# kyle-he/gym-comm

Measured on AMD Instinct MI355X. Metric: env-steps/sec (whole node), higher is better.
Workload: dtype int32

## Files before the change

gym-comm_amd/csrc/oc_step_device.h:

```cpp
#pragma once
#include <hip/hip_runtime.h>

#include <type_traits>

#include "../../include/oc_hip.h"
#include "oc_level_host.h"
#include "oc_policy_device.h"

namespace {

#ifdef OC_STAMPS
#define OC_STAMP(k)                                                                  \
  do {                                                                               \
    unsigned long long t_;                                                           \
    __builtin_amdgcn_sched_barrier(0);                                               \
    asm volatile("s_memtime %0\n\ts_waitcnt lgkmcnt(0)" : "=s"(t_)::"memory");     \
    __builtin_amdgcn_sched_barrier(0);                                               \
    oc_tt[(k)] = t_;                                                                 \
  } while (0)
#define OC_STAMP_PARAM , unsigned long long (&oc_tt)[16]
#define OC_STAMP_PASS , oc_tt
#else
#define OC_STAMP(k) do { } while (0)
#define OC_STAMP_PARAM
// ... 63 lines not shown
#define OC_HDR_LOAD(args) const HdrK L {(args).L}
#endif
#undef OC_KF
#undef OC_KA

constexpr int IW_POS = 0x000000FF, IW_CHOP = 0x00000100, IW_GRP = 0x00000E00, IW_HOLD = 0x00007000,
              IW_SEQ = 0x00FF0000, IW_TSET = 0x0F000000;
template <bool DUP>
constexpr int TS = DUP ? 0x7F000000 : IW_TSET;
template <bool DUP>
constexpr int OBJ = IW_GRP | IW_SEQ | TS<DUP>;
template <bool DUP>
__host__ __device__ constexpr int sig_of_type(int t) { return DUP ? (1 << (24 + 2 * t)) : (1 << (24 + t)); }

template <int A, int M, bool DUP>
struct Env {
  int ap[A], ahp[A];
  int iw[M];
  int t, completed, goalcnt, mctr, err;
  int kn[2];
};
template <int A, int M, bool DUP>
constexpr int state_words() { return A + M + 2 + (DUP ? 2 : 0); }

__device__ __forceinline__ int ipos(int w) { return w & IW_POS; }
__device__ __forceinline__ int ichop(int w) { return (w >> 8) & 1; }
__device__ __forceinline__ int igrp(int w) { return (w >> 9) & 7; }
__device__ __forceinline__ int iseq(int w) { return (w >> 16) & 255; }
__device__ __forceinline__ int itset(int w) { return (w >> 24) & 15; }
__device__ __forceinline__ int bfi(int mask, int a, int b) { return (a & mask) | (b & ~mask); }

template <int A, int M, bool DUP>
__device__ __forceinline__ void unpack(Env<A, M, DUP> &e, const int32_t *w) {
#pragma unroll
  for (int a = 0; a < A; a++) {
    e.ap[a] = w[a] & 255;
    e.ahp[a] = (w[a] >> 8) & 15;
  }
#pragma unroll
  for (int i = 0; i < M; i++) e.iw[i] = w[A + i];
  e.t = (w[0] >> 16) & 0xFFFF;
  e.mctr = (w[1] >> 16) & 255;
  e.err = (w[1] >> 24) & 255;
  e.completed = w[A + M];
  e.goalcnt = w[A + M + 1];
  if constexpr (DUP) e.kn[0] = w[A + M + 2], e.kn[1] = w[A + M + 3];
}

template <int A, int M, bool DUP>
__device__ __forceinline__ void pack(const Env<A, M, DUP> &e, int32_t *w) {
#pragma unroll
  for (int a = 0; a < A; a++) w[a] = e.ap[a] | (e.ahp[a] << 8);
  w[0] |= e.t << 16;
  w[1] |= (e.mctr << 16) | (e.err << 24);
#pragma unroll
  for (int i = 0; i < M; i++) w[A + i] = e.iw[i];
  w[A + M] = e.completed;
  w[A + M + 1] = e.goalcnt;
  if constexpr (DUP) w[A + M + 2] = e.kn[0], w[A + M + 3] = e.kn[1];
}

typedef int P;
constexpr int WAIT_VMCNT0 = 0x0F70;
__device__ __forceinline__ int hide(int v) {
  asm("" : "+v"(v));
  return v;
}
__device__ __forceinline__ P sign_of(int d) { return hide(hide(d) >> 31); }
__device__ __forceinline__ P p_z(int a) { return sign_of((int)((unsigned)a - 1u)); }
__device__ __forceinline__ P p_nz(int a) { return sign_of((int)(0u - (unsigned)a)); }
__device__ __forceinline__ P p_eq(int a, int b) { return sign_of((int)((unsigned)(a ^ b) - 1u)); }
__device__ __forceinline__ P p_ne(int a, int b) { return ~p_eq(a, b); }
__device__ __forceinline__ P p_lt(int a, int b) { return sign_of(a - b); }
__device__ __forceinline__ P p_gt(int a, int b) { return p_lt(b, a); }
__device__ __forceinline__ P p_ge(int a, int b) { return ~p_lt(a, b); }
__device__ __forceinline__ P p_le(int a, int b) { return ~p_lt(b, a); }
__device__ __forceinline__ P p_eq_any(int a, int b) { return hide(a == b ? -1 : 0); }
__device__ __forceinline__ P p_gtu_any(unsigned a, unsigned b) { return hide(a > b ? -1 : 0); }
__device__ __forceinline__ P p_geu_any(unsigned a, unsigned b) { return hide(a >= b ? -1 : 0); }
__device__ __forceinline__ P p_ltu_any(unsigned a, unsigned b) { return hide(a < b ? -1 : 0); }
__device__ __forceinline__ P p_bit(int w, unsigned k) { return hide(__builtin_amdgcn_sbfe(w, k, 1u)); }
__device__ __forceinline__ P p_of(bool uniform) { return uniform ? -1 : 0; }
__device__ __forceinline__ int sel(P m, int a, int b) { return (a & m) | (b & ~m); }

__device__ __forceinline__ int iabs(int v) { return v < 0 ? -v : v; }
__device__ __forceinline__ unsigned sad_u32(unsigned a, unsigned b, unsigned c) {
  unsigned r;
  asm("v_sad_u32 %0, %1, %2, %3" : "=v"(r) : "v"(a), "v"(b), "v"(c));
  return r;
}
__device__ __forceinline__ int manhattan(int p, int q) {
  return (int)sad_u32((unsigned)(p & 15), (unsigned)(q & 15), sad_u32((unsigned)(p >> 4), (unsigned)(q >> 4), 0u));
}
__device__ __forceinline__ int px(int p) { return p & 15; }
__device__ __forceinline__ int py(int p) { return p >> 4; }
__device__ __forceinline__ int dense(const Hdr &L, int p) {
  return __mul24(py(p), L.W() - 16) + p;
}
__device__ __forceinline__ int bit128(uint64_t w0, uint64_t w1, int c) {
  const uint64_t v = (c & 64) ? w1 : w0;
  return (int)((v >> (c & 63)) & 1);
}
__device__ __forceinline__ int item_type(const Hdr &L, int i) { return (L.item_types() >> (4 * i)) & 15; }
__device__ __forceinline__ int cell_type(const Hdr &L, int c) {
  if (!L.planes128())
    return (int)((L.cell_lo(0) >> c) & 1) | ((int)((L.cell_hi(0) >> c) & 1) << 1);
  return bit128(L.cell_lo(0), L.cell_lo(1), c) | (bit128(L.cell_hi(0), L.cell_hi(1), c) << 1);
}

#ifdef OC_SPECIALIZED
constexpr bool OC_BORDER_CLOSED = OC_SPEC_HDR.closed_border != 0;
#else
constexpr bool OC_BORDER_CLOSED = false;
#endif

__device__ __forceinline__ double timestep_of(int t, const RunCfg &R) {
  typedef int v2i __attribute__((ext_vector_type(2)));
  const double dt = (double)t;
  const double q0 = dt * R.inv_T;
  const double r = __builtin_fma(-(double)R.T, q0, dt);
  const v2i q = __builtin_bit_cast(v2i, __builtin_fma(r, R.inv_T, q0));
  const P unlimited = p_of(R.T == 0);
  const int hi0 = 0x7FF00000 | (p_z(t) & 0x00080000);
  v2i out;
  out.x = q.x & ~unlimited;
  out.y = sel(unlimited, hi0, q.y);
  return __builtin_bit_cast(double, out);
}


template <int AUX>
struct RowsT {
  __amdgpu_buffer_rsrc_t rsrc;
  int voff;
  int rowbytes;
  __device__ __forceinline__ RowsT(const void *base, int64_t n, int rows, int64_t i, int elem = 4) {
    rsrc = __builtin_amdgcn_make_buffer_rsrc(const_cast<void *>(base), 0, (int)(n * rows * elem), 0x00020000);
    voff = (int)i * elem;
    rowbytes = (int)n * elem;
  }
  __device__ __forceinline__ int ld(int row) const {
    return __builtin_amdgcn_raw_buffer_load_b32(rsrc, voff, row * rowbytes, 0);
  }
  __device__ __forceinline__ void st(int row, int v) const {
    __builtin_amdgcn_raw_buffer_store_b32(v, rsrc, voff, row * rowbytes, AUX);
  }
  __device__ __forceinline__ void st8(int row, int v) const {
    __builtin_amdgcn_raw_buffer_store_b8((char)v, rsrc, voff, row * rowbytes, AUX);
  }
  __device__ __forceinline__ void st_f64(int row, double v) const {
    typedef int v2i __attribute__((ext_vector_type(2)));
    __builtin_amdgcn_raw_buffer_store_b64(__builtin_bit_cast(v2i, v), rsrc, voff, row * rowbytes, AUX);
  }
  __device__ __forceinline__ int soff(int row) const { return row * rowbytes; }
  __device__ __forceinline__ void st_at(int so, int, int v) const {
    __builtin_amdgcn_raw_buffer_store_b32(v, rsrc, voff, so, AUX);
  }
  __device__ __forceinline__ void st8_at(int so, int, int v) const {
    __builtin_amdgcn_raw_buffer_store_b8((char)v, rsrc, voff, so, AUX);
  }
};
template <int AUX, int N>
struct RowsPreT : RowsT<AUX> {
  int so[N > 0 ? N : 1];
  int row0;
  __device__ __forceinline__ RowsPreT(const RowsT<AUX> &rows, int row0_) : RowsT<AUX>(rows), row0(row0_) {
// ... 215 lines not shown
        d_tile[b] = min(d_tile[b], ld.d_tile[k][b] + manhattan(in.ap[b], (int)L.deliv_pos(k)));
    }
  int nchop = 0;
  int mind[B];
#pragma unroll
  for (int b = 0; b < B; b++) mind[b] = 1 << 20;
#pragma unroll
  for (int f = 0; f < 3; f++)
    if (L.chop_mask(f) != 0) {
      const int open = __popc((int)L.chop_mask(f) & ~completed);
      nchop += open;
#pragma unroll
      for (int b = 0; b < B; b++) mind[b] = open ? min(mind[b], ld.d_chop[f][b]) : mind[b];
    }
  int npairs = (int)L.pair_static_max();
  int minpair = npairs ? MAXP : (1 << 20);
  {
    int cur = MAXP;
#pragma unroll
    for (int k = 0; k < MAX_PAIRLK; k++)
      if (k < (int)L.npairlk()) {
        cur = min(cur, ld.d_pair[k]);
        if ((L.pairlk(k) >> 8) & 1) {
          const bool keep = cur != 0;
          npairs += keep ? 1 : 0;
          minpair = keep ? min(minpair, cur) : minpair;
          cur = MAXP;
        }
      }
  }
  int kq_chop[B], kq_pair;
#pragma unroll
  for (int b = 0; b < B; b++) kq_chop[b] = nchop ? (mind[b] + MAXP) + (nchop - 1) * 2 * MAXP : 0;
  kq_pair = nchop ? npairs * MAXP : (npairs ? minpair + (npairs - 1) * MAXP : 0);
  int kq_del[MAX_DELS][B];
#pragma unroll
  for (int k = 0; k < MAX_DELS; k++)
#pragma unroll
    for (int b = 0; b < B; b++) {
      kq_del[k][b] = 0;
      q.del_direct[k][b] = false;
      if (k < (int)L.ndel()) {
        const int d = ld.d_del[k][b] + manhattan(in.ap[b], in.del_p[k]);
        q.del_direct[k][b] = d == 0;
        kq_del[k][b] = d == 0 ? d_tile[b] : d;
      }
    }
#pragma unroll
  for (int b = 0; b < B; b++) q.q_chop[b] = quotient(kq_chop[b], L, inv_max_path);
  q.q_pair = quotient(kq_pair, L, inv_max_path);
#pragma unroll
  for (int k = 0; k < MAX_DELS; k++)
#pragma unroll
    for (int b = 0; b < B; b++) q.q_del[k][b] = (k < (int)L.ndel()) ? quotient(kq_del[k][b], L, inv_max_path) : 0.0;
  q.nchop = nchop;
  q.npairs = npairs;
  OC_STAMP(4);
}

template <int B>
__device__ __forceinline__ void shaping_sum(const Hdr &L, const ShapeIn<B> &in, const ShapeQ<B> &q,
                                            double &s0, double &s1 OC_STAMP_PARAM) {
  double tot[B];
#pragma unroll
  for (int b = 0; b < B; b++) {
    tot[b] = q.nchop ? q.q_chop[b] : 0.0;
    tot[b] = q.npairs ? tot[b] + q.q_pair : tot[b];
  }
#pragma unroll
  for (int k = 0; k < MAX_DELS; k++)
    if (k < (int)L.ndel()) {
      const bool open = !((in.completed >> L.del_bit(k)) & 1);
#pragma unroll
      for (int b = 0; b < B; b++) {
        const double add = !in.del_has[k] ? 2.0 : (q.del_direct[k][b] ? q.q_del[k][b] : q.q_del[k][b] + 1.0);
        tot[b] = open ? tot[b] + add : tot[b];
      }
    }
  s0 = tot[0];
  s1 = B > 1 ? tot[1] : 0.0;
  OC_STAMP(6);
}

template <int A, int M, bool DUP, int PM, bool FLAT>
__device__ __forceinline__ void env_step(const Hdr &L, const RunCfg &R, const uint8_t *__restrict__ dist,
                                         const uint32_t *__restrict__ probe,
                                         Env<A, M, DUP> &e, const int (&act_in)[A], int &reward, int &done, P &done_p,
                                         int &success, ShapeIn<(A < 2 ? A : 2)> &sin,
                                         ShapeLoads<(A < 2 ? A : 2)> &sld OC_STAMP_PARAM) {
  const int W = L.W(), H = L.H();
  const auto pb = [](int w, unsigned k) -> P {
    if constexpr (PM == 2 && FLAT) return __builtin_amdgcn_sbfe(w, k, 1u);
    return p_bit(w, k);
  };
  e.t = min(e.t + 1, 0xFFFF);
  static_assert(OC_ACT_NOOP == 4 && OC_FLOOR == 0 && OC_COUNTER == 1 && OC_CUTBOARD == 2 && OC_DELIVERY == 3, "codes");

  int act[A], np[A], tgt_p[A];
  P moving[A], t_nonfloor[A], t_deliv[A], t_cutb[A];
#pragma unroll
  for (int a = 0; a < A; a++) {
    int c = act_in[a];
    e.err |= p_gtu_any((unsigned)c, 4u) & OC_ERR_ACTION;
    c = (int)min((unsigned)c, 4u);
    act[a] = c;
    moving[a] = p_ne(c, OC_ACT_NOOP);
    int cell;
    P oob = 0;
    if constexpr (OC_BORDER_CLOSED) {
      constexpr uint64_t STEP = 0x0001FFF010ull;
      const int q = e.ap[a] + (int)(int8_t)(STEP >> (8 * c));
      tgt_p[a] = q;
      cell = dense(L, q);
    } else {
      const int dx = (c == OC_ACT_RIGHT) - (c == OC_ACT_LEFT);
      const int dy = (c == OC_ACT_DOWN) - (c == OC_ACT_UP);
      const int qx = px(e.ap[a]) + dx, qy = py(e.ap[a]) + dy;
      oob = ~(p_ltu_any((unsigned)qx, (unsigned)W) & p_ltu_any((unsigned)qy, (unsigned)H));
      e.err |= oob & OC_ERR_OOB;
      const int tx = min(max(qx, 0), W - 1), ty = min(max(qy, 0), H - 1);
      tgt_p[a] = tx | (ty << 4);
      cell = ty * W + tx;
    }
    P lo, hi;
    if (!L.planes128()) {
      lo = pb((int)(L.cell_lo(0) >> cell), 0);
      hi = pb((int)(L.cell_hi(0) >> cell), 0);
    } else {
      lo = -bit128(L.cell_lo(0), L.cell_lo(1), cell);
      hi = -bit128(L.cell_hi(0), L.cell_hi(1), cell);
    }
    t_nonfloor[a] = lo | hi;
    t_deliv[a] = lo & hi;
    t_cutb[a] = hi & ~lo;
    np[a] = sel(t_nonfloor[a] | oob, e.ap[a], tgt_p[a]);
  }
  P ex[A];
#pragma unroll
  for (int a = 0; a < A; a++) ex[a] = -1;
#pragma unroll
  for (int i = 0; i < A; i++)
#pragma unroll
    for (int j = i + 1; j < A; j++) {
      const P same = p_eq(np[i], np[j]);
      const P i_stays = p_eq(np[i], e.ap[i]) & moving[i];
      const P j_stays = p_eq(np[j], e.ap[j]) & moving[j];
      const P swap = p_eq(e.ap[i], np[j]) & p_eq(e.ap[j], np[i]);
      const P block_i = sel(same, ~i_stays, swap);
      const P block_j = sel(same, i_stays | ~j_stays, swap);
      ex[i] &= ~block_i;
      ex[j] &= ~block_j;
    }

  const P play = p_of(PM == 2 ? R.play != 0 : PM == 1);
#pragma unroll
  for (int a = 0; a < A; a++) {
    const P acting = ex[a] & moving[a];
    const int pa = e.ap[a];
    const int tp = tgt_p[a];
    const int held_g = A == 2 ? hide(e.ahp[a] - 1) : e.ahp[a] - 1;
    const P holding = A == 2 ? ~hide(held_g >> 31) : p_nz(e.ahp[a]);
    const int hold_code = (a + 1) << 12;
    int held_or = 0, tgt_or = 0;
    P mine[M], tgt[M];
#pragma unroll
    for (int i = 0; i < M; i++) {
      const int w = e.iw[i];
      const int u = item_type(L, i) != OC_PLATE ? (w ^ IW_CHOP) : w;
      mine[i] = A == 2 ? pb(w, 12 + a) : p_eq(w & IW_HOLD, hold_code);
      tgt[i] = p_eq(w & (IW_HOLD | IW_POS), tp);
      held_or |= mine[i] & u;
      tgt_or |= tgt[i] & u;
    }
    const P tgt_any = p_nz(tgt_or);
    P held_multi;
    if constexpr (DUP) {
      int nm = 0;
#pragma unroll
      for (int i = 0; i < M; i++) nm -= mine[i];
      held_multi = p_gt(nm, 1);
    } else {
      held_multi = p_nz(held_or & IW_TSET & ((held_or & IW_TSET) - (1 << 24)));
    }
    const P held_fresh = pb(held_or, 8);
    const P any_fresh = pb(held_or | tgt_or, 8);
    const P two_plates = p_nz((held_or & tgt_or) & sig_of_type<DUP>(OC_PLATE));
    const P at_deliv = t_deliv[a];
    const P nf = acting & t_nonfloor[a];
    const P do_move = acting & ~t_nonfloor[a];
    const P nfh = nf & holding & ~at_deliv, nfe = nf & ~holding & ~at_deliv;
    const P do_deliver = nf & holding & at_deliv & held_multi & ~held_fresh;
    const P mergeable = ~(two_plates | any_fresh);
    const P do_merge = nfh & tgt_any & mergeable;
    const P chop_here = t_cutb[a] & ~held_multi & held_fresh & ~play;
    const P do_chop = nfh & ~tgt_any & chop_here;
    const P do_drop = nfh & ~tgt_any & ~chop_here;
    const P chop_there = nfe & tgt_any & play & t_cutb[a] & pb(tgt_or, 8);
    const P do_pick = nfe & tgt_any & ~chop_there & p_of(!((R.allergic >> a) & 1));
    const P put = do_deliver | do_drop | (do_merge & play);
    const P take = (do_merge & ~play) | do_pick;
    const int newg = (int)min((unsigned)held_g, (unsigned)igrp(tgt_or));
    int objf;
    if constexpr (DUP) {
      const int newsig = (held_or & TS<true>) + (tgt_or & TS<true>);
      const int seq4 = M + e.mctr;
      int kf = 0;
#pragma unroll
      for (int j = 0; j < MAX_NAMES; j++)
        if (j < (int)L.nnames()) {
          const P hit = p_eq(newsig >> 24, (int)L.name_sig(j));
          const int sh = 4 * (j & 7);
          const int cur = (e.kn[j >> 3] >> sh) & 15;
          kf = sel(hit, cur, kf);
          const P enter = hit & p_z(cur);
          e.kn[j >> 3] |= enter & do_merge & ((seq4 + 1) << sh);
        }
      const int kseq = sel(p_nz(kf), kf - 1, seq4);
      objf = newsig | (newg << 9) | (((kseq << 4) | seq4) << 16);
    } else {
      objf = ((held_or | tgt_or) & IW_TSET) | (newg << 9) | ((M + e.mctr) << 16);
    }
    if (A > 2) {
      P shared = 0;
#pragma unroll
      for (int b = 0; b < A; b++)
        if (b != a) shared |= p_eq(e.ap[b], pa);
      if (__ballot((shared & do_merge) != 0) != 0) {
        P alias = 0;
#pragma unroll
        for (int j = 0; j < M; j++) {
          const int w = e.iw[j];
          alias |= p_nz(w & IW_HOLD) & p_ne(w & IW_HOLD, hold_code) & p_eq(ipos(w), pa) &
                   p_z((w ^ held_or) & TS<DUP>) & p_gt(w & IW_SEQ, held_or & IW_SEQ);
        }
        e.err |= shared & do_merge & alias & OC_ERR_ALIAS;
      }
    }
    const int mask_m = ((do_move | put) & IW_POS) | (put & IW_HOLD) | (do_merge & OBJ<DUP>) | (do_chop & IW_CHOP);
    const int mask_t = (take & (IW_POS | IW_HOLD)) | (do_merge & OBJ<DUP>) | (chop_there & IW_CHOP);
    const int val_m = tp | IW_CHOP | objf;
    const int val_t = pa | hold_code | objf | IW_CHOP;
#pragma unroll
    for (int i = 0; i < M; i++) {
      const int selm = (mine[i] & mask_m) | (tgt[i] & mask_t);
      e.iw[i] = bfi(selm, sel(mine[i], val_m, val_t), e.iw[i]);
    }
    e.ap[a] = sel(do_move, tp, pa);
    e.ahp[a] = sel(take, newg + 1, e.ahp[a]) & ~put;
    e.mctr -= do_merge;
  }

  constexpr int B = A < 2 ? A : 2;
#pragma unroll
  for (int b = 0; b < B; b++) sin.ap[b] = e.ap[b];
  if constexpr (DUP) {
#pragma unroll
    for (int f = 0; f < 3; f++) {
      sin.chop_p[f] = 0;
      if (L.chop_mask(f) != 0) {
        bool cand[M];
#pragma unroll
        for (int i = 0; i < M; i++) cand[i] = ((L.food_items(f) >> i) & 1) && !(e.iw[i] & IW_CHOP);
        int has;
        sin.chop_p[f] = pyset_first<M>(L, probe, e.iw, cand, has);
      }
    }
  }
  {
    int ipb[M];
#pragma unroll
    for (int i = 0; i < M; i++) ipb[i] = ipos(e.iw[i]);
    shaping_issue_pos<B, M, DUP>(L, dist, sin, ipb, sld);
    __builtin_amdgcn_sched_barrier(0);
  }
  OC_STAMP(2);
  const int d0 = (int)L.deliv_pos(0);
  int present = 0, at_delivery = 0;
  P rep_ok[M];
#pragma unroll
  for (int i = 0; i < M; i++) {
    const int w = e.iw[i];
    const P rep = p_eq(w & IW_GRP, i << 9);
    const P lone_fresh = item_type(L, i) != OC_PLATE
                             ? p_eq(w & (TS<DUP> | IW_CHOP), sig_of_type<DUP>(item_type(L, i))) : 0;
    rep_ok[i] = rep & ~lone_fresh;
    if constexpr (!DUP) {
      const int b = rep_ok[i] & (1 << itset(w));
      present |= b;
      at_delivery |= p_eq(ipos(w), d0) & b;
    }
  }
  int cnt_mask = 0, del_mask = 0, newly;
  if constexpr (DUP) {
    int rose = 0;
#pragma unroll
    for (int g = 0; g < MAX_GOALS; g++)
      if (g < (int)L.ngoal()) {
        int cnt = 0;
        P hasd = 0;
        P m[M];
#pragma unroll
        for (int i = 0; i < M; i++) {
          m[i] = rep_ok[i] & p_eq(e.iw[i] & TS<true>, (int)L.goal_sig(g) << 24);
          P seen = 0;
#pragma unroll
          for (int j = 0; j < i; j++) seen |= m[j] & p_eq(ipos(e.iw[j]), ipos(e.iw[i]));
          cnt -= m[i] & ~seen;
          hasd |= m[i] & p_eq(ipos(e.iw[i]), d0);
        }
        cnt = min(cnt, 3);
        const int old = (e.goalcnt >> (2 * g)) & 3;
        rose |= p_gt(cnt, old) & (int)L.goal_nd(g);
        cnt_mask |= cnt << (2 * g);
        del_mask |= hasd & (int)L.goal_dl(g);
      }
    newly = rose;
  } else {
#pragma unroll
    for (int g = 0; g < MAX_GOALS; g++) {
      if (g < (int)L.ngoal()) {
        cnt_mask |= pb(present, L.goal_tset(g)) & (int)L.goal_nd(g);
        del_mask |= pb(at_delivery, L.goal_tset(g)) & (int)L.goal_dl(g);
      }
    }
    newly = cnt_mask & ~e.goalcnt;
  }
  reward = __popc(newly) + 3 * __popc(del_mask);
  e.completed |= newly | del_mask;
  e.goalcnt = cnt_mask;
  P timeout;
  if constexpr (FLAT) timeout = p_ge(e.t, R.T != 0 ? (int)R.T : 0x10000);
  else timeout = R.T != 0 ? p_ge(e.t, R.T) : 0;
  const P all_delivered = p_eq_any(del_mask, (int)L.deliver_mask());
  done_p = hide(timeout | all_delivered);
  done = done_p & 1;
  success = (~timeout & all_delivered) & 1;

// ... 232 lines not shown
  row += 16;
#pragma unroll
  for (int k = 0; k < S / 2; k++) OUTV(row + 2 * k, lp.vo1, (e.completed >> lp.shp[k]) & 1);
  if constexpr ((S & 1) != 0) OUTV(row + S - 1, out.voff, (e.completed >> lp.sh_odd) & 1);
  row += S;
#pragma unroll
  for (int j = 0; j < CPP; j++) OUTV(row + j, lp.voA, loc[j]);
  row += 4;
  OUTV(row, lp.vo1, p_nz(vhp) & ~lp.hi & 1);
  row += 2;
  const int commv = sel(lp.hi, comm1, comm0);
#define COMM_ROWS(CC_)                                                                              \
  do {                                                                                              \
    _Pragma("unroll") for (int c = 0; c < (CC_); c++) OUTV(row + c, lp.voC, commv == c ? 1 : 0);   \
    asm volatile("");                                                                               \
  } while (0)
  if (C == 2) {
    COMM_ROWS(2);
  } else {
    int Cx = C;
    asm("" : "+s"(Cx));
    switch (Cx) {
      case 1: COMM_ROWS(1); break;
      case 3: COMM_ROWS(3); break;
      case 4: COMM_ROWS(4); break;
      default: {
        int so = out.soff(row);
        for (int c = 0; c < C; c++, row++, so += out.rowbytes) {
          if (OT == 1) out.st8_at(so, row, comm0 == c ? 1 : 0);
          else if (OT == 2) out.st_at(so, row, __builtin_bit_cast(int, (float)(comm0 == c ? 1 : 0)));
          else out.st_at(so, row, comm0 == c ? 1 : 0);
        }
        for (int c = 0; c < C; c++, row++, so += out.rowbytes) {
          if (OT == 1) out.st8_at(so, row, comm1 == c ? 1 : 0);
          else if (OT == 2) out.st_at(so, row, __builtin_bit_cast(int, (float)(comm1 == c ? 1 : 0)));
          else out.st_at(so, row, comm1 == c ? 1 : 0);
        }
      }
    }
  }
#undef COMM_ROWS
#undef OUTV
}
#endif

__device__ __forceinline__ int wave_sum_lane63(int v) {
  v += __builtin_amdgcn_update_dpp(0, v, 0x111, 0xF, 0xF, true);
  v += __builtin_amdgcn_update_dpp(0, v, 0x112, 0xF, 0xF, true);
  v += __builtin_amdgcn_update_dpp(0, v, 0x114, 0xF, 0xF, true);
  v += __builtin_amdgcn_update_dpp(0, v, 0x118, 0xF, 0xF, true);
  v += __builtin_amdgcn_update_dpp(0, v, 0x142, 0xA, 0xF, false);
  v += __builtin_amdgcn_update_dpp(0, v, 0x143, 0xC, 0xF, false);
  return v;
}

struct MetricsSlot {
  unsigned long long *p;
  __device__ __forceinline__ MetricsSlot(int64_t *metrics, int64_t thread_index) {
    const int lane = threadIdx.x & 63;
    p = (metrics != nullptr && lane < 6)
            ? (unsigned long long *)metrics + (thread_index >> 6) * OC_MET_COUNT + lane
            : nullptr;
  }
  __device__ __forceinline__ void add(bool has_metrics, bool valid, int done, int success, int reward,
                                      int completed_bits, bool err) {
    if (!has_metrics) return;
    const P ok = hide(valid ? -1 : 0), fin = ok & -done;
    const int a = (ok & reward) | ((fin & __popc(completed_bits)) << 12);
    const int b = (ok & 1) | (fin & (1 << 7)) | (ok & -success & (1 << 14)) | (ok & hide(err ? -1 : 0) & (1 << 21));
    const unsigned ta = (unsigned)__builtin_amdgcn_readlane(wave_sum_lane63(a), 63);
    const unsigned tb = (unsigned)__builtin_amdgcn_readlane(wave_sum_lane63(b), 63);
    constexpr unsigned OFF = 0u | 7u << 5 | 14u << 10 | 0u << 15 | 12u << 20 | 21u << 25;
    constexpr unsigned WID = 7u | 7u << 5 | 7u << 10 | 12u << 15 | 12u << 20 | 7u << 25;
    static_assert(64 * OC_MAX_SUBTASKS < (1 << 12) && 64 * (OC_MAX_SUBTASKS + 3 * MAX_DELS) < (1 << 12),
                  "wave sums must fit their 12-bit fields");
    static_assert(OC_MET_ENV_STEPS == 0 && OC_MET_EPISODES == 1 && OC_MET_SUCCESSES == 2 &&
                  OC_MET_REWARD_SUM == 3 && OC_MET_COMPLETED_SUM == 4 && OC_MET_ERRORS == 5, "slot order");
    const unsigned lane = threadIdx.x & 63, k5 = (lane < 6 ? lane : 0) * 5;
    const unsigned off = (OFF >> k5) & 31, wid = (WID >> k5) & 31;
    const unsigned src = (lane == OC_MET_REWARD_SUM || lane == OC_MET_COMPLETED_SUM) ? ta : tb;
    const int v = (int)((src >> off) & ((1u << wid) - 1u));
    if (p) __hip_atomic_fetch_add(p, (unsigned long long)v, __ATOMIC_RELAXED, __HIP_MEMORY_SCOPE_AGENT);
  }
};

struct Tables {
  const uint8_t *dist;
  const uint8_t *counters;
  const uint32_t *probe;
};

template <bool LDS>
__device__ __forceinline__ Tables stage_tables(const void *__restrict__ tables, int n16, int quot_bytes) {
  Tables tb;
  if constexpr (LDS) {
    extern __shared__ uint4 oc_lds[];
    const uint4 *src = (const uint4 *)tables;
    const int i0 = threadIdx.x, i1 = i0 + blockDim.x, i2 = i1 + blockDim.x, i3 = i2 + blockDim.x;
    uint4 t0 = make_uint4(0, 0, 0, 0), t1 = t0, t2 = t0, t3 = t0;
    if (i0 < n16) t0 = src[i0];
    if (i1 < n16) t1 = src[i1];
    if (i2 < n16) t2 = src[i2];
    if (i3 < n16) t3 = src[i3];
    for (int idx = threadIdx.x + 4 * blockDim.x; idx < n16; idx += blockDim.x) oc_lds[idx] = src[idx];
    if (i0 < n16) oc_lds[i0] = t0;
    if (i1 < n16) oc_lds[i1] = t1;
    if (i2 < n16) oc_lds[i2] = t2;
    if (i3 < n16) oc_lds[i3] = t3;
    __syncthreads();
    tb.dist = (const uint8_t *)oc_lds + quot_bytes;
    tb.counters = (const uint8_t *)oc_lds + (n16 * 16 - OC_MAX_COUNTERS);
    tb.probe = (const uint32_t *)((const uint8_t *)oc_lds + (n16 * 16 - OC_MAX_COUNTERS - 4 * OC_MAX_CELLS));
  } else {
    tb.dist = (const uint8_t *)tables;
    tb.counters = (const uint8_t *)tables + (n16 * 16 - OC_MAX_COUNTERS);
    tb.probe = (const uint32_t *)((const uint8_t *)tables + (n16 * 16 - OC_MAX_COUNTERS - 4 * OC_MAX_CELLS));
  }
  return tb;
}

struct MapRef {
  const LevelHdr &L;
  const RunCfg &R;
  const void *const &tables;
  const int32_t &n16;
};
struct LaunchMap {
  MapRef mp;
  __device__ __forceinline__ MapRef ref() const { return mp; }
  __device__ __forceinline__ MapRef ref_behind_loads() const { return mp; }
};

__device__ __forceinline__ uint32_t pcg32(uint32_t &state) {
  state = state * 747796405u + 2891336453u;
  const uint32_t w = ((state >> ((state >> 28u) + 4u)) ^ state) * 277803737u;
  return (w >> 22u) ^ w;
}

template <int A, int M, int WS>
__device__ __forceinline__ void place_items_from(const Hdr &L, const Tables &tb, const int32_t *placement,
                                                 bool use_rng, uint32_t &st, int64_t n, int64_t i,
                                                 int32_t (&w)[WS]) {
  if (L.nscatter() == 0) return;
  int pos[M];
#pragma unroll
  for (int k = 0; k < M; k++) pos[k] = w[A + k] & 255;
  if (use_rng) {
    unsigned long long taken = 0;
    for (int k = 0; k < (int)L.nscatter(); k++) {
      int idx = 0;
      bool ok = false;
      for (int attempt = 0; attempt < 64 && !ok; attempt++) {
        idx = (int)__umulhi(pcg32(st), L.ncounters());
        ok = !((taken >> idx) & 1);
      }
      for (int c = 0; c < (int)L.ncounters() && !ok; c++) {
        idx = c;
        ok = !((taken >> idx) & 1);
      }
      taken |= 1ull << idx;
      const int cell = tb.counters[idx];
      const int item = (int)L.scatter_item(k & 3);
#pragma unroll
      for (int m = 0; m < M; m++) pos[m] = (item == m) ? cell : pos[m];
    }
  } else if (placement != nullptr) {
// ... 273 lines not shown
  if (i >= p.n) return;
  if (p.mask != nullptr && p.mask[i] == 0) return;
  constexpr int WS = state_words<A, M, DUP>();
  const Tables tb = stage_tables<false>(tables, n16, 0);
  int32_t w[WS];
#pragma unroll
  for (int r = 0; r < WS; r++) w[r] = L.init_words(r);
  place_items<A, M, WS>(L, tb, p.placement, p.rng, p.n, i, w);
#pragma unroll
  for (int r = 0; r < WS; r++) p.state[(int64_t)r * p.n + i] = w[r];
}

template <int A, int M, bool DUP>
__global__ void __launch_bounds__(256) k_reset(const ResetArgs p) {
  reset_body<A, M, DUP>(p.L, p.tables, p.n16, p);
}

__global__ void __launch_bounds__(256) k_random_actions(uint32_t *rng, int32_t *move_row, int32_t *comm_row,
                                                        uint32_t num_comm, int64_t n) {
  const int64_t i = (int64_t)blockIdx.x * blockDim.x + threadIdx.x;
  if (i >= n) return;
  uint32_t st = rng[i];
  move_row[i] = (int32_t)__umulhi(pcg32(st), 4u);
  comm_row[i] = (int32_t)__umulhi(pcg32(st), num_comm);
  rng[i] = st;
}

struct MultiArgs {
  LevelHdr L;
  RunCfg R;
  const void *tables;
  int32_t n16, quot_bytes;
  int32_t *state;
  int32_t *comm;
  const int32_t *actions;
  void *obs;
  double *timestep;
  double *reward;
  int32_t *done;
  int32_t *sparse;
  int64_t *metrics;
  const int32_t *placement;
  uint32_t *rng;
  oc_step_opts opt;
  int64_t n;
  int32_t auto_reset;
  oc_wrap_cfg cfg;
  oc_step_policy pol[2];
  int32_t pol_ksteps;
  unsigned long long *timeline;
  int64_t timeline_stride;
};

constexpr int DUTY_STATE = 1, DUTY_SHAPE = 2, DUTY_OBS0 = 4, DUTY_OBS1 = 8, DUTY_ALL = 15;

template <int ROWS>
__device__ __forceinline__ float *pol_lds_feat() {
  __shared__ float a[2 * ROWS * 64];
  return a;
}
__device__ __forceinline__ float *pol_lds_ts() {
  __shared__ float t[64];
  return t;
}

template <int M, bool LDS, int OT, bool WT, bool DUP, int XO, int DUTY, bool SPLIT, bool POL = false, int LN = 1,
          typename ARGS = MultiArgs, typename MAPS = LaunchMap>
__device__ __forceinline__ void multi_step_body(int32_t *const state_, const int32_t *const actions_,
                                                int32_t *const comm_, int64_t *const metrics_,
                                                const int32_t n_, const int32_t block_, const void *const ego_src_,
                                                const void *const alt_src_, const ARGS &p, const MAPS &maps) {
  constexpr int A = 2;
  constexpr bool D_STATE = (DUTY & DUTY_STATE) != 0, D_SHAPE = (DUTY & DUTY_SHAPE) != 0;
  using Out = RowsT<WT ? AUX_WT : 0>;
#ifdef OC_SPECIALIZED
  constexpr int POL_ROWS = (POL && SPLIT) ? 22 + OC_SPEC_HDR.S + 8 : 1;
#else
  constexpr int POL_ROWS = 1;
#endif
  static_assert(LN == 1 || (SPLIT && XO == 0 && !POL && !LDS && DUTY != DUTY_ALL), "lane-split: the plain four-way split only");
  constexpr int EPW = 64 / LN;
  const int i = SPLIT ? (int)blockIdx.x * EPW + (int)(threadIdx.x & (EPW - 1))
                      : (int)blockIdx.x * (block_ & 0xFFFF) + (int)threadIdx.x;
  constexpr bool PART0_ONLY = LN > 1 && (DUTY & (DUTY_OBS0 | DUTY_OBS1)) == 0;
  const bool valid = PART0_ONLY ? (i < (int)n_ && (int)(threadIdx.x & 63) < EPW) : i < (int)n_;
  const bool ego_from_pairs = XO != 0 && ((block_ >> 16) & 1), alt_from_pairs = XO != 0 && ((block_ >> 17) & 1),
             alt_from_rng = XO != 0 && ((block_ >> 18) & 1), pairs64 = XO != 0 && ((block_ >> 19) & 1);
#ifdef OC_STAMPS
  unsigned long long oc_tt[16];
  for (int k = 0; k < 16; k++) oc_tt[k] = 0;
#endif
  OC_STAMP(0);
  Tables tb;
  if constexpr (LDS) tb = stage_tables<true>(maps.ref().tables, maps.ref().n16, p.quot_bytes);
  MetricsSlot slot(metrics_, i);
  int reward = 0, done = 0, success = 0, comp = 0;
  bool err = false;
  constexpr int POL_MINE = (DUTY == DUTY_OBS0) ? 0 : (DUTY == DUTY_OBS1) ? 2 : (DUTY == DUTY_STATE) ? 1 : 3;
  constexpr int POL_VIEWER = POL_MINE >> 1;
  [[maybe_unused]] ocpol::Weights pol_w;
  if constexpr (POL && SPLIT) {
    ocpol::load_weights(pol_w, p.pol[POL_VIEWER].w1, p.pol[POL_VIEWER].w2, p.pol[POL_VIEWER].b2,
                        (int)threadIdx.x & 63, p.pol_ksteps);
  }
  if (valid) {
    constexpr int WS = state_words<A, M, DUP>();
    const Out st(state_, n_, WS, i), cm(comm_, n_, 2, i);
    int32_t w[WS];
#pragma unroll
    for (int r = 0; r < WS; r++) w[r] = st.ld(r);
    typedef int v2i __attribute__((ext_vector_type(2)));
    typedef int v4i __attribute__((ext_vector_type(4)));
    v4i eq = {0, 0, 0, 0}, aq = {0, 0, 0, 0};
    v2i er = {0, 0}, ar = {0, 0};
    uint32_t alt_rs = 0;
    if constexpr (XO != 0) {
      const auto desc = [&](const void *base, bool on, int bytes) {
        return __builtin_amdgcn_make_buffer_rsrc(const_cast<void *>(base), 0, on ? bytes : 0, 0x00020000);
      };
      const int sh = pairs64 ? 4 : 3;
      const __amdgpu_buffer_rsrc_t d_er = desc(actions_, !ego_from_pairs, (int)n_ * 16),
                                   d_ar = desc(actions_, !alt_from_pairs && !alt_from_rng, (int)n_ * 16),
                                   d_eq = desc(ego_src_, ego_from_pairs, (int)n_ << sh),
                                   d_aq = desc(alt_src_, alt_from_pairs && !alt_from_rng, (int)n_ << sh),
                                   d_rs = desc(alt_src_, alt_from_rng, (int)n_ * 4);
      const int off4 = i << 2, offq = i << sh, row = (int)n_ * 4;
      eq = (v4i)__builtin_amdgcn_raw_buffer_load_b128(d_eq, offq, 0, 0);
      aq = (v4i)__builtin_amdgcn_raw_buffer_load_b128(d_aq, offq, 0, 0);
      alt_rs = (uint32_t)__builtin_amdgcn_raw_buffer_load_b32(d_rs, off4, 0, 0);
      er.x = __builtin_amdgcn_raw_buffer_load_b32(d_er, off4, 0, 0);
      er.y = __builtin_amdgcn_raw_buffer_load_b32(d_er, off4, row, 0);
      ar.x = __builtin_amdgcn_raw_buffer_load_b32(d_ar, off4, 2 * row, 0);
      ar.y = __builtin_amdgcn_raw_buffer_load_b32(d_ar, off4, 3 * row, 0);
    } else {
      const Rows ac(actions_, n_, 4, i);
      er.x = ac.ld(0), er.y = ac.ld(1);
      ar.x = ac.ld(2), ar.y = ac.ld(3);
    }
    const MapRef mp = maps.ref_behind_loads();
    const Hdr L {mp.L};
    if constexpr (!LDS) tb = stage_tables<false>(mp.tables, mp.n16, 0);
    asm volatile("" ::"s"(tb.dist), "s"(p.obs), "s"(p.timestep), "s"(p.reward), "s"(p.done),
                 "s"(p.sparse), "s"(p.auto_reset), "s"(mp.R.inv_T), "s"(mp.R.inv_max_path));
    if constexpr (XO != 0) asm volatile("" ::"s"(p.opt.ep_return), "s"(p.opt.ep_length));
#if defined(OC_SPECIALIZED) && !defined(OC_SPEC_GEOMETRY)
    asm volatile("" ::"s"(L.W()), "s"(L.ncells()), "s"(L.max_path()), "s"(L.cell_lo(0)), "s"(L.cell_hi(0)),
                 "s"(L.deliv_pos(0)));
#endif
    double ep_ret = 0.0;
    int ep_len = 0, prev_done = 0;
    if (XO != 0 && p.opt.ep_return != nullptr) {
      const Rows er(p.opt.ep_return, n_, 1, i, 8);
      ep_ret = __builtin_bit_cast(double, (v2i)__builtin_amdgcn_raw_buffer_load_b64(er.rsrc, er.voff, 0, 0));
      ep_len = Rows(p.opt.ep_length, n_, 1, i).ld(0);
      prev_done = Rows(p.done, n_, 1, i).ld(0);
    }
    Env<A, M, DUP> e;
    unpack<A, M, DUP>(e, w);
    const int C = p.cfg.obs.num_comm;
    const int F = 22 + L.S() + 2 * C;
    const Out ob(p.obs, p.n, 2 * F, i, OT == 1 ? 1 : 4);
    constexpr bool OBS_ONLY = SPLIT && (DUTY == DUTY_OBS0 || DUTY == DUTY_OBS1);
#ifdef OC_TS_OBS1
    constexpr int TS_DUTY = POL ? DUTY_OBS0 : DUTY_OBS1;
#else
    constexpr int TS_DUTY = DUTY_OBS0;
#endif
#ifdef OC_SPECIALIZED
    constexpr int NPRE_ALL = 22 + (int)OC_SPEC_HDR.S + 8;
    constexpr int NPRE = (OBS_ONLY && !POL && XO == 0) ? (NPRE_ALL < 40 ? NPRE_ALL : 40) : 0;
#else
    constexpr int NPRE = 0;
#endif
    const ObsSlots slots(mp.R, NPRE != 0);
    const RowsPreT<WT ? AUX_WT : 0, NPRE> obp(ob, DUTY == DUTY_OBS1 ? F : 0);
    if constexpr (NPRE != 0) asm volatile("" ::"s"(ob.rsrc));
#ifdef OC_SPECIALIZED
    using Parts = std::conditional_t<(LN > 1 && OBS_ONLY), LaneParts<(LN > 1 ? LN : 2)>, NoParts>;
    [[maybe_unused]] const Parts parts(ob, slots, C);
#endif
    const Out tso(p.timestep, p.n, 1, i, 8);
    if constexpr (NPRE != 0 && DUTY == TS_DUTY) asm volatile("" ::"s"(tso.rsrc), "v"(tso.voff));
    uint32_t place_rs = 0;
    if constexpr (SPLIT) {
      if (L.nscatter() != 0 && p.rng != nullptr) place_rs = (uint32_t)Rows(p.rng, n_, 1, i).ld(0);
      if constexpr (XO != 0)
        asm volatile("s_waitcnt vmcnt(0)\n\ts_barrier" : "+v"(eq), "+v"(aq), "+v"(er), "+v"(ar), "+v"(alt_rs)::"memory");
      else asm volatile("s_waitcnt vmcnt(0)\n\ts_barrier" ::: "memory");
      __builtin_amdgcn_s_waitcnt(WAIT_VMCNT0);
      if constexpr (NPRE != 0) __builtin_amdgcn_sched_barrier(0);
    } else if constexpr (XO != 0) {
      asm volatile("" : "+v"(eq), "+v"(aq), "+v"(er), "+v"(ar), "+v"(alt_rs));
    }
    int ego_mv = er.x, ego_cm = er.y, alt_mv = ar.x, alt_cm = ar.y;
    if constexpr (XO != 0) {
      const auto narrow = [](int lo, int hi) { return lo | ~p_eq_any(hi, lo >> 31); };
      if (pairs64) {
        ego_mv |= narrow(eq.x, eq.y), ego_cm |= narrow(eq.z, eq.w);
        alt_mv |= narrow(aq.x, aq.y), alt_cm |= narrow(aq.z, aq.w);
      } else {
        ego_mv |= eq.x, ego_cm |= eq.y;
        alt_mv |= aq.x, alt_cm |= aq.y;
      }
    }
    if (alt_from_rng) {
      alt_mv = (int)__umulhi(pcg32(alt_rs), 4u);
      alt_cm = (int)__umulhi(pcg32(alt_rs), (uint32_t)p.cfg.obs.num_comm);
      if (!SPLIT || D_STATE) {
        Rows(alt_src_, n_, 1, i).st(0, (int)alt_rs);
        if (p.opt.alt_played != nullptr) {
          const Rows ap(p.opt.alt_played, n_, 2, i);
          ap.st(0, alt_mv);
          ap.st(1, alt_cm);
        }
      }
    }
    OC_STAMP(1);
    const bool cfg_comm_on = XO == 2 ? p.cfg.communication_on != 0 : true, cfg_ego_led = XO == 2 ? p.cfg.ego_led != 0 : false;
    const int cfg_can_move = XO == 2 ? p.cfg.can_move_mask : 3, cfg_ego_idx = XO == 2 ? p.cfg.ego_agent_idx : 0;
    const int cfg_blind = XO == 2 ? p.cfg.obs.blind_mask : 0;
    const unsigned NC = (unsigned)p.cfg.obs.num_comm;
    const bool ego_talks = cfg_comm_on, alt_talks = cfg_comm_on && !cfg_ego_led;
    const P ego_cm_bad = p_geu_any((unsigned)ego_cm, NC), alt_cm_bad = p_geu_any((unsigned)alt_cm, NC);
    const P bad_cm = (p_of(ego_talks) & ego_cm_bad) | (p_of(alt_talks) & alt_cm_bad);
    const int c0 = ego_talks ? (ego_cm | ego_cm_bad) : -1;
    const int c1 = alt_talks ? (alt_cm | alt_cm_bad) : -1;
    if constexpr (D_STATE) {
      cm.st(0, c0);
      cm.st(1, c1);
    }
    const P bad_mv = p_gtu_any((unsigned)ego_mv, 3u) | p_gtu_any((unsigned)alt_mv, 3u);
    const int em = (cfg_can_move & 1) ? (int)min((unsigned)ego_mv, 4u) : OC_ACT_NOOP;
    const int am = (cfg_can_move & 2) ? (int)min((unsigned)alt_mv, 4u) : OC_ACT_NOOP;
    int act[A];
    act[0] = cfg_ego_idx == 0 ? em : am;
    act[1] = cfg_ego_idx == 0 ? am : em;
    const int err_before = e.err;
    P done_p = 0;
    e.err |= (bad_mv | bad_cm) & OC_ERR_ACTION;
    ShapeIn<2> sin;
    ShapeLoads<2> sld;
    env_step<A, M, DUP, XO == 2 ? 2 : 0, SPLIT>(L, mp.R, tb.dist, tb.probe, e, act, reward, done, done_p, success, sin, sld OC_STAMP_PASS);
    comp = e.completed;
    err = e.err != err_before;
    if constexpr (D_STATE) {
      Out(p.done, p.n, 1, i).st(0, done);
#ifndef OC_STAMPS
      if (p.sparse != nullptr) Out(p.sparse, p.n, 1, i).st(0, reward);
#endif
    }
    if constexpr (DUTY != DUTY_SHAPE) {
      if ((DUTY & (DUTY_OBS0 | DUTY_OBS1)) == 0 && L.nscatter() == 0) {
        pack<A, M, DUP>(e, w);
        const P fresh = done_p & p_of(p.auto_reset != 0);
#pragma unroll
        for (int r = 0; r < WS; r++) w[r] = sel(fresh, L.init_words(r), w[r]);
      } else if (OBS_ONLY && L.nscatter() == 0) {
        int32_t w0[WS];
#pragma unroll
        for (int r = 0; r < WS; r++) w0[r] = L.init_words(r);
        Env<A, M, DUP> e0;
        unpack<A, M, DUP>(e0, w0);
        const P fresh = done_p & p_of(p.auto_reset != 0);
#pragma unroll
        for (int a = 0; a < A; a++) e.ap[a] = sel(fresh, e0.ap[a], e.ap[a]), e.ahp[a] = sel(fresh, e0.ahp[a], e.ahp[a]);
#pragma unroll
        for (int k = 0; k < M; k++) e.iw[k] = sel(fresh, e0.iw[k], e.iw[k]);
        e.t = sel(fresh, e0.t, e.t);
        e.completed = sel(fresh, e0.completed, e.completed);
      } else if (done && p.auto_reset) {
#pragma unroll
        for (int r = 0; r < WS; r++) w[r] = L.init_words(r);
        if constexpr (SPLIT) {
          place_items_from<A, M, WS>(L, tb, p.placement, p.rng != nullptr, place_rs, p.n, i, w);
          if (D_STATE && L.nscatter() != 0 && p.rng != nullptr) p.rng[i] = place_rs;
        } else {
          place_items<A, M, WS>(L, tb, p.placement, p.rng, p.n, i, w);
        }
        unpack<A, M, DUP>(e, w);
      } else {
        pack<A, M, DUP>(e, w);
      }
    }
    if constexpr (D_STATE) {
#pragma unroll
      for (int r = 0; r < WS; r++) st.st(r, w[r]);
    }
    constexpr bool TS_MINE = OBS_ONLY ? DUTY == TS_DUTY : (DUTY & DUTY_OBS0) != 0;
    [[maybe_unused]] double tsd = 0.0;
    if constexpr (TS_MINE && OBS_ONLY && !POL) tsd = timestep_of(e.t, mp.R);
    if constexpr (TS_MINE && OBS_ONLY && !POL) tso.st_f64(0, tsd);
    ShapeQ<2> sq;
    if constexpr (D_SHAPE) shaping_lookup<2>(L, mp.R.inv_max_path, sin, sld, sq OC_STAMP_PASS);
    const bool ego_blind = cfg_blind & 1;
    if constexpr (POL && SPLIT) {
      const int ln = (int)threadIdx.x & 63;
      if constexpr ((DUTY & DUTY_OBS0) != 0) {
        const RowsLdsT<WT ? AUX_WT : 0, OT> obl(ob, pol_lds_feat<POL_ROWS>(), 0, ln);
        env_obs<A, M, DUP, OT>(L, mp.R, slots, e, 0, p.cfg.obs.fow_radius, cfg_blind & 1, ego_blind, C, c0, c1, obl, 0);
        const double tsd = timestep_of(e.t, mp.R);
        Out(p.timestep, p.n, 1, i, 8).st_f64(0, tsd);
        pol_lds_ts()[ln] = (float)tsd;
      }
      if constexpr ((DUTY & DUTY_OBS1) != 0) {
        const RowsLdsT<WT ? AUX_WT : 0, OT> obl(ob, pol_lds_feat<POL_ROWS>() + POL_ROWS * 64, F, ln);
        env_obs<A, M, DUP, OT>(L, mp.R, slots, e, 1, p.cfg.obs.fow_radius, (cfg_blind >> 1) & 1, ego_blind, C, c0, c1, obl, F);
      }
    } else {
#ifdef OC_SPECIALIZED
      if constexpr (LN > 1) {
        if constexpr (DUTY == DUTY_OBS0) env_obs_lanes<A, M, DUP, OT, LN>(L, parts, e, 0, p.cfg.obs.fow_radius, C, c0, c1, obp, 0);
        if constexpr (DUTY == DUTY_OBS1) env_obs_lanes<A, M, DUP, OT, LN>(L, parts, e, 1, p.cfg.obs.fow_radius, C, c0, c1, obp, F);
      } else
#endif
      {
        if constexpr ((DUTY & DUTY_OBS0) != 0)
          env_obs<A, M, DUP, OT>(L, mp.R, slots, e, 0, p.cfg.obs.fow_radius, cfg_blind & 1, ego_blind, C, c0, c1, obp, 0);
        if constexpr ((DUTY & DUTY_OBS1) != 0)
          env_obs<A, M, DUP, OT>(L, mp.R, slots, e, 1, p.cfg.obs.fow_radius, (cfg_blind >> 1) & 1, ego_blind, C, c0, c1, obp, F);
      }
      if constexpr (TS_MINE && !OBS_ONLY) tso.st_f64(0, timestep_of(e.t, mp.R));
    }
    OC_STAMP(5);
    if constexpr (D_SHAPE) {
      double s0, s1;
      shaping_sum<2>(L, sin, sq, s0, s1 OC_STAMP_PASS);
      const double shaped = ((double)reward - s0) - s1;
      Out(p.reward, p.n, 1, i, 8).st_f64(0, shaped);
      if (XO != 0 && p.opt.ep_return != nullptr) {
        Out(p.opt.ep_return, p.n, 1, i, 8).st_f64(0, prev_done ? shaped : ep_ret + shaped);
        Out(p.opt.ep_length, p.n, 1, i).st(0, prev_done ? 1 : ep_len + 1);
      }
    }
  }
  OC_STAMP(7);
  if constexpr (D_STATE) slot.add(metrics_ != nullptr, valid, done, success, reward, comp, err);
  OC_STAMP(8);
  if constexpr (POL) {
    static_assert(XO != 0, "the fused policies belong to the variants with action sources");
    if constexpr (SPLIT) asm volatile("s_waitcnt lgkmcnt(0)\n\ts_barrier" ::: "memory");
    else asm volatile("s_waitcnt vmcnt(0)" ::: "memory");
    const int lane = (int)threadIdx.x & 63;
    const Hdr L {maps.ref().L};
    const int C = p.cfg.obs.num_comm, F = 22 + L.S() + 2 * C;
    const uint32_t n32 = (uint32_t)n_;
    constexpr int ELEM = OT == 1 ? 1 : 4;
#pragma unroll
    for (int v = 0; v < 2; v++)
#pragma unroll
      for (int q = 0; q < 2; q++) {
        if (SPLIT && (2 * v + q) != POL_MINE) continue;
        const int64_t env0 = (int64_t)(i & ~63) + 32 * q + (lane & 31);
        const bool ok = env0 < n_;
        const uint32_t env = (uint32_t)(ok ? env0 : n_ - 1);
        const void *rows = (const char *)p.obs + (size_t)v * F * n_ * ELEM;
        int32_t *pairs = (int32_t *)const_cast<void *>(v == 0 ? ego_src_ : alt_src_);
        if constexpr (SPLIT) {
          const int col = 32 * q + (lane & 31);
          ocpol::policy_pass<OT, 4, true, true>(rows, n32, env, ok, lane, p.pol[v].w1, p.pol[v].w2, p.pol[v].b2,
                                                p.pol[v].rng, pairs, nullptr, pol_lds_ts()[col], F, C, p.pol_ksteps,
                                                pol_lds_feat<POL_ROWS>() + v * POL_ROWS * 64, col, &pol_w);
        } else {
          ocpol::policy_pass<OT, 4>(rows, n32, env, ok, lane, p.pol[v].w1, p.pol[v].w2, p.pol[v].b2, p.pol[v].rng,
                                    pairs, nullptr, (float)p.timestep[env], F, C, p.pol_ksteps);
        }
      }
  }
#ifdef OC_STAMPS
  if ((threadIdx.x & 63) == 0 && p.sparse != nullptr) {
    long long *dbg = (long long *)p.sparse + ((int64_t)blockIdx.x * (blockDim.x >> 6) + (threadIdx.x >> 6)) * 16;
    for (int k = 0; k < 16; k++) dbg[k] = (long long)oc_tt[k];
  }
#endif
}

template <int M, bool LDS, int OT, bool WT, bool DUP, int XO, int SP, bool POL = false, int LN = 1>
__global__ void __launch_bounds__(256) k_multi_step(int32_t *const state_, const int32_t *const actions_,
                                                    int32_t *const comm_, int64_t *const metrics_,
                                                    const int32_t n_, const int32_t block_,
                                                    const void *const ego_src_, const void *const alt_src_,
                                                    const MultiArgs p) {
  static_assert(SP == 1 || SP == 2 || SP == 4, "waves per 64 envs");
  static_assert(SP != 2 || !POL, "the fused policies need the four-wave split");
  static_assert(SP == 1 || !LDS, "the split launch reads the tables from global memory");
  static_assert(LN == 1 || (SP == 4 && XO == 0 && !POL), "lanes per env: the plain four-way split only");
  OC_TL_BEGIN();
#ifdef OC_SPECIALIZED
  const MultiArgs &pk = p;
#else
  struct KernArgs { int32_t *a; const int32_t *b; int32_t *c; int64_t *d; int32_t n, blk; const void *e, *f; MultiArgs p; };
  [[maybe_unused]] const MultiArgs &pk = *reinterpret_cast<const MultiArgs *>(
      reinterpret_cast<const char *>((const void *)__builtin_amdgcn_kernarg_segment_ptr()) + offsetof(KernArgs, p));
#endif
#define OC_BODY(duty) multi_step_body<M, LDS, OT, WT, DUP, XO, (duty), true, POL, LN>(state_, actions_, comm_, metrics_, n_, block_, ego_src_, alt_src_, pk, LaunchMap{{pk.L, pk.R, pk.tables, pk.n16}})
  if constexpr (SP == 1) {
    multi_step_body<M, LDS, OT, WT, DUP, XO, DUTY_ALL, false, POL>(state_, actions_, comm_, metrics_, n_, block_, ego_src_, alt_src_, p,
                                                                   LaunchMap{{p.L, p.R, p.tables, p.n16}});
  } else {
    const int role = __builtin_amdgcn_readfirstlane((int)threadIdx.x >> 6);
    if constexpr (SP == 2) {
      if (role == 0) OC_BODY(DUTY_STATE | DUTY_OBS0);
      else OC_BODY(DUTY_SHAPE | DUTY_OBS1);
    } else {
      if (role == 0) OC_BODY(DUTY_OBS0);
      else if (role == 1) OC_BODY(DUTY_OBS1);
      else if (role == 2) OC_BODY(DUTY_STATE);
      else OC_BODY(DUTY_SHAPE);
    }
  }
#undef OC_BODY
  OC_TL_END(p.timeline, p.timeline_stride, LN);
}


#if defined(OC_SPECIALIZED) && !defined(OC_SPEC_GEOMETRY)
struct MapRecord {
  LevelHdr L;
  RunCfg R;
  int64_t tab_off;
// ... 101 lines not shown
```

Measured before the change: 1.609 billion.

## Split state and shaping duties across wave halves with per-half agent work

In multi-lane (LN>1) split kernels, the state-duty wave now lets both 32-lane halves do useful work: each half stores alternate state words and comm values via part_sel, halving per-lane stores. The shaping-duty wave computes shaping for one agent per half and exchanges sums with permlane32_swap. Metrics reduction uses a DPP-based per-half sum, replacing two full-wave reductions. This adds cross-lane shuffles and relies on both halves holding identical env state, and it drops the OC_TS_OBS1 option.

```diff
diff --git a/gym-comm_amd/csrc/oc_step_device.h b/gym-comm_amd/csrc/oc_step_device.h
--- a/gym-comm_amd/csrc/oc_step_device.h
+++ b/gym-comm_amd/csrc/oc_step_device.h
@@ -169,6 +169,9 @@
 __device__ __forceinline__ P p_bit(int w, unsigned k) { return hide(__builtin_amdgcn_sbfe(w, k, 1u)); }
 __device__ __forceinline__ P p_of(bool uniform) { return uniform ? -1 : 0; }
 __device__ __forceinline__ int sel(P m, int a, int b) { return (a & m) | (b & ~m); }
+__device__ __forceinline__ int part_sel(int part1, int part0) {
+  return __builtin_amdgcn_inverse_ballot_w64(0xFFFFFFFF00000000ull) ? part1 : part0;
+}
 
 __device__ __forceinline__ int iabs(int v) { return v < 0 ? -v : v; }
 __device__ __forceinline__ unsigned sad_u32(unsigned a, unsigned b, unsigned c) {
@@ -550,12 +553,11 @@
   OC_STAMP(6);
 }
 
-template <int A, int M, bool DUP, int PM, bool FLAT>
+template <int A, int M, bool DUP, int PM, bool FLAT, int SB = (A < 2 ? A : 2)>
 __device__ __forceinline__ void env_step(const Hdr &L, const RunCfg &R, const uint8_t *__restrict__ dist,
                                          const uint32_t *__restrict__ probe,
                                          Env<A, M, DUP> &e, const int (&act_in)[A], int &reward, int &done, P &done_p,
-                                         int &success, ShapeIn<(A < 2 ? A : 2)> &sin,
-                                         ShapeLoads<(A < 2 ? A : 2)> &sld OC_STAMP_PARAM) {
+                                         int &success, ShapeIn<SB> &sin, ShapeLoads<SB> &sld OC_STAMP_PARAM) {
   const int W = L.W(), H = L.H();
   const auto pb = [](int w, unsigned k) -> P {
     if constexpr (PM == 2 && FLAT) return __builtin_amdgcn_sbfe(w, k, 1u);
@@ -718,9 +720,14 @@
     e.mctr -= do_merge;
   }
 
-  constexpr int B = A < 2 ? A : 2;
-#pragma unroll
-  for (int b = 0; b < B; b++) sin.ap[b] = e.ap[b];
+  constexpr int B = SB;
+  static_assert(B == (A < 2 ? A : 2) || (B == 1 && A == 2), "shaping agents per lane");
+  if constexpr (B == 1 && A == 2) {
+    sin.ap[0] = part_sel(e.ap[1], e.ap[0]);
+  } else {
+#pragma unroll
+    for (int b = 0; b < B; b++) sin.ap[b] = e.ap[b];
+  }
   if constexpr (DUP) {
 #pragma unroll
     for (int f = 0; f < 3; f++) {
@@ -1119,6 +1126,28 @@
     const int v = (int)((src >> off) & ((1u << wid) - 1u));
     if (p) __hip_atomic_fetch_add(p, (unsigned long long)v, __ATOMIC_RELAXED, __HIP_MEMORY_SCOPE_AGENT);
   }
+  __device__ __forceinline__ void add_parts(bool has_metrics, bool valid, int done, int success, int reward,
+                                            int completed_bits, bool err) {
+    if (!has_metrics) return;
+    const P ok = hide(valid ? -1 : 0), fin = ok & -done;
+    const int a = (ok & reward) | ((fin & __popc(completed_bits)) << 12);
+    const int b = (ok & 1) | (fin & (1 << 7)) | (ok & -success & (1 << 14)) | (ok & hide(err ? -1 : 0) & (1 << 21));
+    int v = part_sel(b, a);
+    v += __builtin_amdgcn_update_dpp(0, v, 0x111, 0xF, 0xF, true);
+    v += __builtin_amdgcn_update_dpp(0, v, 0x112, 0xF, 0xF, true);
+    v += __builtin_amdgcn_update_dpp(0, v, 0x114, 0xF, 0xF, true);
+    v += __builtin_amdgcn_update_dpp(0, v, 0x118, 0xF, 0xF, true);
+    v += __builtin_amdgcn_update_dpp(0, v, 0x142, 0xA, 0xF, false);
+    const unsigned ta = (unsigned)__builtin_amdgcn_readlane(v, 31);
+    const unsigned tb = (unsigned)__builtin_amdgcn_readlane(v, 63);
+    constexpr unsigned OFF = 0u | 7u << 5 | 14u << 10 | 0u << 15 | 12u << 20 | 21u << 25;
+    constexpr unsigned WID = 7u | 7u << 5 | 7u << 10 | 12u << 15 | 12u << 20 | 7u << 25;
+    const unsigned lane = threadIdx.x & 63, k5 = (lane < 6 ? lane : 0) * 5;
+    const unsigned off = (OFF >> k5) & 31, wid = (WID >> k5) & 31;
+    const unsigned src = (lane == OC_MET_REWARD_SUM || lane == OC_MET_COMPLETED_SUM) ? ta : tb;
+    const int val = (int)((src >> off) & ((1u << wid) - 1u));
+    if (p) __hip_atomic_fetch_add(p, (unsigned long long)val, __ATOMIC_RELAXED, __HIP_MEMORY_SCOPE_AGENT);
+  }
 };
 
 struct Tables {
@@ -1558,8 +1587,8 @@
   constexpr int EPW = 64 / LN;
   const int i = SPLIT ? (int)blockIdx.x * EPW + (int)(threadIdx.x & (EPW - 1))
                       : (int)blockIdx.x * (block_ & 0xFFFF) + (int)threadIdx.x;
-  constexpr bool PART0_ONLY = LN > 1 && (DUTY & (DUTY_OBS0 | DUTY_OBS1)) == 0;
-  const bool valid = PART0_ONLY ? (i < (int)n_ && (int)(threadIdx.x & 63) < EPW) : i < (int)n_;
+  constexpr bool HW_STATE = LN > 1 && DUTY == DUTY_STATE, HW_SHAPE = LN > 1 && DUTY == DUTY_SHAPE;
+  const bool valid = i < (int)n_;
   const bool ego_from_pairs = XO != 0 && ((block_ >> 16) & 1), alt_from_pairs = XO != 0 && ((block_ >> 17) & 1),
              alt_from_rng = XO != 0 && ((block_ >> 18) & 1), pairs64 = XO != 0 && ((block_ >> 19) & 1);
 #ifdef OC_STAMPS
@@ -1637,11 +1666,7 @@
     const int F = 22 + L.S() + 2 * C;
     const Out ob(p.obs, p.n, 2 * F, i, OT == 1 ? 1 : 4);
     constexpr bool OBS_ONLY = SPLIT && (DUTY == DUTY_OBS0 || DUTY == DUTY_OBS1);
-#ifdef OC_TS_OBS1
-    constexpr int TS_DUTY = POL ? DUTY_OBS0 : DUTY_OBS1;
-#else
     constexpr int TS_DUTY = DUTY_OBS0;
-#endif
 #ifdef OC_SPECIALIZED
     constexpr int NPRE_ALL = 22 + (int)OC_SPEC_HDR.S + 8;
     constexpr int NPRE = (OBS_ONLY && !POL && XO == 0) ? (NPRE_ALL < 40 ? NPRE_ALL : 40) : 0;
@@ -1655,6 +1680,12 @@
     using Parts = std::conditional_t<(LN > 1 && OBS_ONLY), LaneParts<(LN > 1 ? LN : 2)>, NoParts>;
     [[maybe_unused]] const Parts parts(ob, slots, C);
 #endif
+    constexpr int NPW = (WS + 1) / 2;
+    [[maybe_unused]] int st_vo = 0;
+    if constexpr (HW_STATE) {
+      st_vo = st.voff + part_sel(st.rowbytes, 0);
+      asm volatile("" : "+v"(st_vo));
+    }
     const Out tso(p.timestep, p.n, 1, i, 8);
     if constexpr (NPRE != 0 && DUTY == TS_DUTY) asm volatile("" ::"s"(tso.rsrc), "v"(tso.voff));
     uint32_t place_rs = 0;
@@ -1701,7 +1732,9 @@
     const P bad_cm = (p_of(ego_talks) & ego_cm_bad) | (p_of(alt_talks) & alt_cm_bad);
     const int c0 = ego_talks ? (ego_cm | ego_cm_bad) : -1;
     const int c1 = alt_talks ? (alt_cm | alt_cm_bad) : -1;
-    if constexpr (D_STATE) {
+    if constexpr (HW_STATE) {
+      __builtin_amdgcn_raw_buffer_store_b32(part_sel(c1, c0), cm.rsrc, st_vo, 0, WT ? AUX_WT : 0);
+    } else if constexpr (D_STATE) {
       cm.st(0, c0);
       cm.st(1, c1);
     }
@@ -1714,9 +1747,10 @@
     const int err_before = e.err;
     P done_p = 0;
     e.err |= (bad_mv | bad_cm) & OC_ERR_ACTION;
-    ShapeIn<2> sin;
-    ShapeLoads<2> sld;
-    env_step<A, M, DUP, XO == 2 ? 2 : 0, SPLIT>(L, mp.R, tb.dist, tb.probe, e, act, reward, done, done_p, success, sin, sld OC_STAMP_PASS);
+    constexpr int SB = HW_SHAPE ? 1 : 2;
+    ShapeIn<SB> sin;
+    ShapeLoads<SB> sld;
+    env_step<A, M, DUP, XO == 2 ? 2 : 0, SPLIT, SB>(L, mp.R, tb.dist, tb.probe, e, act, reward, done, done_p, success, sin, sld OC_STAMP_PASS);
     comp = e.completed;
     err = e.err != err_before;
     if constexpr (D_STATE) {
@@ -1725,8 +1759,18 @@
       if (p.sparse != nullptr) Out(p.sparse, p.n, 1, i).st(0, reward);
 #endif
     }
+    [[maybe_unused]] int32_t wp[NPW];
     if constexpr (DUTY != DUTY_SHAPE) {
-      if ((DUTY & (DUTY_OBS0 | DUTY_OBS1)) == 0 && L.nscatter() == 0) {
+      if (HW_STATE && L.nscatter() == 0) {
+        pack<A, M, DUP>(e, w);
+        const P fresh = done_p & p_of(p.auto_reset != 0);
+        const P fresh1 = part_sel(fresh, 0), fresh0 = part_sel(0, fresh);
+#pragma unroll
+        for (int k = 0; k < NPW; k++) {
+          if (2 * k + 1 < WS) wp[k] = sel(fresh1, L.init_words(2 * k + 1), sel(fresh0, L.init_words(2 * k), part_sel(w[2 * k + 1], w[2 * k])));
+          else wp[k] = sel(fresh, L.init_words(2 * k), w[2 * k]);
+        }
+      } else if ((DUTY & (DUTY_OBS0 | DUTY_OBS1)) == 0 && L.nscatter() == 0) {
         pack<A, M, DUP>(e, w);
         const P fresh = done_p & p_of(p.auto_reset != 0);
 #pragma unroll
@@ -1758,7 +1802,15 @@
         pack<A, M, DUP>(e, w);
       }
     }
-    if constexpr (D_STATE) {
+    if constexpr (HW_STATE) {
+      if (L.nscatter() != 0) {
+#pragma unroll
+        for (int k = 0; k < NPW; k++) wp[k] = 2 * k + 1 < WS ? part_sel(w[2 * k + 1], w[2 * k]) : w[2 * k];
+      }
+#pragma unroll
+      for (int k = 0; k < NPW; k++)
+        __builtin_amdgcn_raw_buffer_store_b32(wp[k], st.rsrc, 2 * k + 1 < WS ? st_vo : st.voff, 2 * k * st.rowbytes, WT ? AUX_WT : 0);
+    } else if constexpr (D_STATE) {
 #pragma unroll
       for (int r = 0; r < WS; r++) st.st(r, w[r]);
     }
@@ -1766,8 +1818,8 @@
     [[maybe_unused]] double tsd = 0.0;
     if constexpr (TS_MINE && OBS_ONLY && !POL) tsd = timestep_of(e.t, mp.R);
     if constexpr (TS_MINE && OBS_ONLY && !POL) tso.st_f64(0, tsd);
-    ShapeQ<2> sq;
-    if constexpr (D_SHAPE) shaping_lookup<2>(L, mp.R.inv_max_path, sin, sld, sq OC_STAMP_PASS);
+    ShapeQ<SB> sq;
+    if constexpr (D_SHAPE) shaping_lookup<SB>(L, mp.R.inv_max_path, sin, sld, sq OC_STAMP_PASS);
     const bool ego_blind = cfg_blind & 1;
     if constexpr (POL && SPLIT) {
       const int ln = (int)threadIdx.x & 63;
@@ -1800,7 +1852,15 @@
     OC_STAMP(5);
     if constexpr (D_SHAPE) {
       double s0, s1;
-      shaping_sum<2>(L, sin, sq, s0, s1 OC_STAMP_PASS);
+      shaping_sum<SB>(L, sin, sq, s0, s1 OC_STAMP_PASS);
+      if constexpr (HW_SHAPE) {
+        typedef unsigned v2u __attribute__((ext_vector_type(2)));
+        const v2u own = __builtin_bit_cast(v2u, s0);
+        const v2u lo = __builtin_amdgcn_permlane32_swap(own.x, own.x, false, false);
+        const v2u hi = __builtin_amdgcn_permlane32_swap(own.y, own.y, false, false);
+        s0 = __builtin_bit_cast(double, (v2u){lo.x, hi.x});
+        s1 = __builtin_bit_cast(double, (v2u){lo.y, hi.y});
+      }
       const double shaped = ((double)reward - s0) - s1;
       Out(p.reward, p.n, 1, i, 8).st_f64(0, shaped);
       if (XO != 0 && p.opt.ep_return != nullptr) {
@@ -1810,7 +1870,8 @@
     }
   }
   OC_STAMP(7);
-  if constexpr (D_STATE) slot.add(metrics_ != nullptr, valid, done, success, reward, comp, err);
+  if constexpr (HW_STATE) slot.add_parts(metrics_ != nullptr, valid, done, success, reward, comp, err);
+  else if constexpr (D_STATE) slot.add(metrics_ != nullptr, valid, done, success, reward, comp, err);
   OC_STAMP(8);
   if constexpr (POL) {
     static_assert(XO != 0, "the fused policies belong to the variants with action sources");
```

Result: slower. 1.561 billion (-3.0%).
